# gersteinlab/LESSeq

Measured on AMD Instinct MI355X. Metric: MRF reads/sec through count+solve, higher is better.
Workload: dtype int32 coordinates / u64 counters (count), f64 (EM); 1 GPU; BASELINE configs[2]: 100M synthetic 100bp reads over 50k mixed events (SE/RI/A5SS/A3SS/MXE/AFE/ALE/T3), 24 chromosomes; events=50000

## Files before the change

### lesseq_amd/csrc/lsq_count.hip

```cpp
#include "lsq_device.hpp"
#include <hip/hip_ext.h>

namespace {

#ifndef LSQ_COUNT_BLOCK
#define LSQ_COUNT_BLOCK 256
#endif
constexpr int COUNT_BLOCK = LSQ_COUNT_BLOCK;
constexpr unsigned long long BASES_MASK = (1ull << 40) - 1;

#ifdef LSQ_DEV
#define ABL(args, bits) ((((args).ablate) & (bits)) != 0u)
#else
#define ABL(args, bits) false
#endif


struct CountArgs {
	const BucketDesc *buckets;
	const unsigned char *images;
	const TieRec *ties;
	const unsigned char *strand_rank;
	const char *read_names; const unsigned long long *read_name_off;
	const char *gene_names; const unsigned *gene_name_off;
// ... 1247 lines not shown
                     const unsigned *look1, const unsigned *look2, const size_t B, const unsigned long long grid, const SharePlanCosts &pc, unsigned long long *cut) {
	if (!(pc.weighted && pn1 && pn2 && look1 && look2)) { plan_share_cuts_seg(so, visited_kind, B, nullptr, nullptr, nullptr, nullptr, 0, grid, pc, cut); return; }
	std::vector<unsigned long long> x; std::vector<unsigned char> kind; std::vector<unsigned> looks, bseg(B + 1, 0);
	for (size_t b = 0; b < B; ++b) {
		bseg[b] = (unsigned)kind.size();
		const unsigned long long ns = so[b + 1] - so[b];
		if (!ns) continue;
		const bool visited = visited_kind[b] != 0;
		const unsigned long long n1 = visited ? std::min(pn1[b], ns) : 0, n2 = visited ? std::min(pn2[b], ns - n1) : 0;
		if (n1) { x.push_back(so[b]); kind.push_back(0); looks.push_back(look1[b]); }
		if (n2) { x.push_back(so[b] + n1); kind.push_back(1); looks.push_back(look2[b]); }
		if (ns - n1 - n2) { x.push_back(so[b] + n1 + n2); kind.push_back(2); looks.push_back(0); }
	}
	bseg[B] = (unsigned)kind.size();
	x.push_back(B ? so[B] : 0);
	plan_share_cuts_seg(so, visited_kind, B, x.data(), kind.data(), looks.data(), bseg.data(), kind.size(), grid, pc, cut);
}

int run_count(lsq_ctx *c) {
	const lsq_events &E = *c->E;
	const size_t n_cls = E.n_cls_total;
	const int M = E.n_methods;
	hipStream_t st_em = nullptr;
	const int set = c->flip ^ 1, other = c->flip;
	hipStream_t st = c->opt_two_count_streams ? c->stream_count2[set] : c->stream;
	if (c->mark_recorded2[set]) HIP_TRY(hipStreamWaitEvent(st, c->ev_mark2[set], 0));
	HIP_TRY(hipMemsetAsync(c->counters.p + (size_t)other * c->counters_per_set, 0, c->counters_per_set * sizeof(unsigned long long), c->stream_em2[other]));
	HIP_TRY(hipEventRecord(c->ev_mark2[other], c->stream_em2[other]));
	c->mark_recorded2[other] = true;
	select_counter_set(c, set);
	st_em = c->stream_em;
	c->fast_launched = 0;
	struct Cleanup { CountArgs A; unsigned long long n_pn; int m; };
	std::vector<Cleanup> cleanups;
	bool counted_signalled = false;
	if (c->time_events) HIP_TRY(hipEventRecord(c->ev0, st));
	const unsigned generic_tables_bytes = (std::max<unsigned>(E.max_lds_bytes, 16) + 15u) & ~15u;
	const unsigned tables_bytes = generic_tables_bytes;
	double max_skew = 0.0;
	for (int m = 0; m < M; ++m) max_skew = std::max(max_skew, c->reads[m].skew);
	const unsigned cap = c->opt_wg_per_cu >= 0 ? (unsigned)c->opt_wg_per_cu : (c->em.small_places >= c->em.opt_flat_min && max_skew < 4.0 ? 5u : 0u);
	const unsigned lds_bytes = std::max(tables_bytes + WAVES * WAVE_QUEUE_WORDS * 16, cap ? 160u * 1024u / (cap + 1u) + 16u : 0u);
	if (lds_bytes > 160 * 1024) return fail(LSQ_E_UNSUPPORTED, "bucket tables + read tile exceed the CU's LDS");
	bool all_compact = true;
	for (int m = 0; m < M; ++m) if (c->reads[m].total_slots && !c->reads[m].compact) all_compact = false;
	const int p1w = !all_compact ? 2 : (c->opt_reads_per_look ? (c->opt_reads_per_look == 8 ? 4 : 2) : (cap != 0 && cap <= 5 ? 4 : 2));
	const void *const fn_wide = (const void *)lsq_count_fast_kernel<false, 2>;
	const void *const fn_compact = p1w == 4 ? (const void *)lsq_count_fast_kernel<true, 4> : (const void *)lsq_count_fast_kernel<true, 2>;
	c->last_reads_per_look = 2u * (unsigned)p1w;
	if (lds_bytes > 64 * 1024) {
		HIP_TRY(hipFuncSetAttribute(fn_wide, hipFuncAttributeMaxDynamicSharedMemorySize, (int)lds_bytes));
		HIP_TRY(hipFuncSetAttribute(fn_compact, hipFuncAttributeMaxDynamicSharedMemorySize, (int)lds_bytes));
		HIP_TRY(hipFuncSetAttribute((const void *)lsq_count_generic_kernel, hipFuncAttributeMaxDynamicSharedMemorySize, (int)lds_bytes));
// ... 80 lines not shown
		A.exc = mr.exc.p + (size_t)set * mr.exc_cap; A.exc_count = c->exc_count.p + 2 * m; A.exc_cap = (unsigned)mr.exc_cap;
		A.dbg = c->dbg.p; A.bar = c->dbg.p + 16 + m;
		A.wg_trace = nullptr;
		const unsigned long long n_pn = mr.pn_strand.n;
		A.n_pn = n_pn;
		const unsigned workers_per_cu = 2;
		A.n_workers = (unsigned)std::min<unsigned long long>((n_pn + COUNT_BLOCK - 1) / COUNT_BLOCK, (unsigned long long)c->n_cu * workers_per_cu);
#ifdef LSQ_DEV
		if (c->dev_ablate & 32768u) A.n_workers = 0;
#endif
		if (c->has_fast) {
			if (c->time_events) HIP_TRY(hipEventRecord(c->evf0[m], st));
			const bool last_streaming = m == M - 1 && !c->has_generic && !c->time_events;
			const dim3 fgrid((unsigned)grid + A.n_workers);
#ifdef LSQ_DEV
			if (c->dev_ablate & 4194304u) {
				if (c->wg_trace.n < 4ull * fgrid.x) { int rc = c->wg_trace.alloc(4ull * fgrid.x); if (rc) return rc; }
				HIP_TRY(hipMemsetAsync(c->wg_trace.p, 0, 4ull * fgrid.x * sizeof(unsigned long long), st));
				c->wg_trace_n = fgrid.x; c->wg_trace_workers = A.n_workers;
				A.wg_trace = c->wg_trace.p;
			}
#endif
			void *kargs[] = {(void *)&A};
			HIP_TRY(hipExtLaunchKernel(mr.compact ? fn_compact : fn_wide, fgrid, dim3(COUNT_BLOCK), kargs, lds_bytes, st, nullptr, last_streaming ? c->ev_counted2[set] : nullptr, 0));
			if (last_streaming) counted_signalled = true;
			if (c->time_events) HIP_TRY(hipEventRecord(c->evf1[m], st));
			c->fast_launched |= 1 << m;
			cleanups.push_back({A, n_pn, m});
		}
		if (c->has_generic) {
			hipLaunchKernelGGL(lsq_count_generic_kernel, dim3((unsigned)grid), dim3(COUNT_BLOCK), generic_tables_bytes, st, A);
			HIP_TRY(hipGetLastError());
		}
	}
	if (c->time_events) HIP_TRY(hipEventRecord(c->ev1, st));
	c->count_timed = c->time_events;
	if (!counted_signalled) HIP_TRY(hipEventRecord(c->ev_counted2[set], st));
	HIP_TRY(hipStreamWaitEvent(st_em, c->ev_counted2[set], 0));
	const unsigned rgrid = std::max(16u, (unsigned)c->n_cu);
	if (c->recount_args.n < 2 * (size_t)LSQ_MAX_METHODS * sizeof(CountArgs)) {
		int rc = c->recount_args.alloc(2 * (size_t)LSQ_MAX_METHODS * sizeof(CountArgs));
		if (rc) return rc;
		c->recount_args_host.assign(2 * (size_t)LSQ_MAX_METHODS * sizeof(CountArgs), 0);
	}
	for (const Cleanup &u : cleanups) {
		const size_t slot = ((size_t)set * LSQ_MAX_METHODS + (size_t)u.m) * sizeof(CountArgs);
		if (memcmp(c->recount_args_host.data() + slot, &u.A, sizeof(CountArgs)) != 0) {
			memcpy(c->recount_args_host.data() + slot, &u.A, sizeof(CountArgs));
			HIP_TRY(hipMemcpyAsync(c->recount_args.p + slot, c->recount_args_host.data() + slot, sizeof(CountArgs), hipMemcpyHostToDevice, st_em));
		}
		const CountArgs *dA = reinterpret_cast<const CountArgs *>(c->recount_args.p + slot);
		hipLaunchKernelGGL(lsq_count_cleanup_kernel, dim3(c->opt_cleanup_grid ? c->opt_cleanup_grid : rgrid), dim3(256), 0, st_em, dA, c->opt_recount ? 1 : 0, u.n_pn,
		                   (const ExcEntry *)u.A.exc, (const unsigned *)u.A.exc_count, u.A.exc_cap);
		HIP_TRY(hipGetLastError());
	}
	return LSQ_OK;
}

}

extern "C" {

int lsq_count_status(lsq_ctx *c, uint32_t *exceptions, uint32_t *recounted) LSQ_API_TRY {
	if (!c) return fail(LSQ_E_ARG, "null context");
	if (!c->counted) return fail(LSQ_E_STATE, "lsq_count must come first");
	HIP_TRY(hipSetDevice(c->device));
// ... 78 lines not shown
```

### lesseq_amd/csrc/lsq_device.hip

```cpp
#include "lsq_device.hpp"
#include <chrono>
#include <thread>

namespace lsq {

int upload_strand_ranks(lsq_ctx *c) {
	const auto &names = c->E->strands.names;
	if (names.size() > 256) return fail(LSQ_E_RANGE, "more than 256 distinct strand strings");
	std::vector<int> order(names.size());
	std::iota(order.begin(), order.end(), 0);
	std::sort(order.begin(), order.end(), [&](int a, int b) { return names[a] < names[b]; });
	std::vector<uint8_t> rank(256, 0);
	for (size_t r = 0; r < order.size(); ++r) rank[order[r]] = (uint8_t)r;
	int rc = c->strand_rank.upload(rank.data(), 256, c->stream);
	if (rc) return rc;
	HIP_TRY(hipStreamSynchronize(c->stream));
	return LSQ_OK;
}

static hipError_t wait_for_stream(hipStream_t s) {
	const auto t0 = std::chrono::steady_clock::now();
	for (;;) {
		const hipError_t e = hipStreamQuery(s);
		if (e != hipErrorNotReady) return e;
		if (std::chrono::steady_clock::now() - t0 > std::chrono::milliseconds(2)) return hipStreamSynchronize(s);
	}
}

int ensure_lanes(lsq_ctx *c) {
	if (c->lanes_thread.joinable()) c->lanes_thread.join();
	if (c->lanes_status) return fail(c->lanes_status, "%s", c->lanes_error.c_str());
	return LSQ_OK;
}

int sync_all(lsq_ctx *c) {
	{ const int rc = ensure_lanes(c); if (rc) return rc; }
	HIP_TRY(wait_for_stream(c->stream_count2[0]));
	HIP_TRY(wait_for_stream(c->stream_count2[1]));
	HIP_TRY(wait_for_stream(c->stream_em2[0]));
	HIP_TRY(wait_for_stream(c->stream_em2[1]));
	HIP_TRY(wait_for_stream(c->stream));
	return LSQ_OK;
}

void select_counter_set(lsq_ctx *c, int set) {
	unsigned long long *base = c->counters.p + (size_t)set * c->counters_per_set;
	const size_t per = c->cnt.n;
	c->flip = set;
	c->stream_em = c->stream_em2[set];
	c->theta.p = c->theta2[set].p; c->theta.n = c->theta2[set].n;
	c->logll.p = c->logll2[set].p; c->logll.n = c->logll2[set].n;
	c->iters.p = c->iters2[set].p; c->iters.n = c->iters2[set].n;
	c->flags.p = c->flags2[set].p; c->flags.n = c->flags2[set].n;
	c->cnt.p = base;
	c->bases.p = base + per;
	c->exc_count.p = reinterpret_cast<unsigned *>(base + 2 * per);
	c->dbg.p = base + 2 * per + LSQ_MAX_METHODS;
}

void note_overflow(lsq_ctx *c, const std::vector<unsigned> &h) {
	for (int m = 0; m < c->E->n_methods; ++m) {
		if (!h[2 * (size_t)m + 1] || c->overflow_logged[m]) continue;
		c->overflow_logged[m] = true;
		if (c->opt_recount) continue;
		warn("read file %d: the exception list overflowed (%u pairs for %zu entries); every read of the file was counted again on the device. "
		     "Tables are complete; raise lsq_ctx_set_option \"exception_capacity\" to avoid the second pass", m, h[2 * (size_t)m], c->reads[m].exc_cap);
	}
}

}

extern "C" {

int lsq_ctx_create(int device_id, lsq_ctx **out) { return lsq_ctx_create_with(device_id, 0u, out); }

int lsq_ctx_create_with(int device_id, unsigned flags, lsq_ctx **out) LSQ_API_TRY {
	if (!out) return fail(LSQ_E_ARG, "null argument");
	const bool timing = getenv("LSQ_CLI_TIMING") != nullptr;
	auto t_last = std::chrono::steady_clock::now();
	auto mark = [&](const char *what) {
		if (!timing) return;
		const auto t = std::chrono::steady_clock::now();
		fprintf(stderr, "[timing]     %-32s %.3f s\n", what, std::chrono::duration<double>(t - t_last).count());
		t_last = t;
	};
	int n = 0;
	hipError_t e = hipGetDeviceCount(&n);
	mark("context: runtime start-up");
	if (e != hipSuccess || n <= 0) return fail(LSQ_E_DEVICE, "no HIP device available (%s)", e == hipSuccess ? "device count 0" : hipGetErrorString(e));
	if (device_id < 0 || device_id >= n) return fail(LSQ_E_ARG, "device %d out of range (%d devices)", device_id, n);
	HIP_TRY(hipSetDevice(device_id));
	hipDeviceProp_t prop;
	HIP_TRY(hipGetDeviceProperties(&prop, device_id));
	if (strncmp(prop.gcnArchName, "gfx950", 6) != 0)
		return fail(LSQ_E_DEVICE, "device %d is %s; this library carries gfx950 code only", device_id, prop.gcnArchName);
	mark("context: device selected");
	std::unique_ptr<lsq_ctx> c(new lsq_ctx);
	c->device = device_id;
	c->n_cu = prop.multiProcessorCount;
	HIP_TRY(hipStreamCreateWithFlags(&c->stream, hipStreamNonBlocking));
	HIP_TRY(hipEventCreate(&c->evt0)); HIP_TRY(hipEventCreate(&c->evt1));
	mark("context: upload stream");
	lsq_ctx *cp = c.get();
	auto make_lanes = [cp]() -> int {
		HIP_TRY(hipSetDevice(cp->device));
		for (int l = 0; l < 2; ++l) {
			HIP_TRY(hipStreamCreateWithFlags(&cp->stream_em2[l], hipStreamNonBlocking));
			HIP_TRY(hipStreamCreateWithFlags(&cp->stream_count2[l], hipStreamNonBlocking));
			HIP_TRY(hipEventCreateWithFlags(&cp->ev_counted2[l], hipEventDisableTiming));
			HIP_TRY(hipEventCreateWithFlags(&cp->ev_mark2[l], hipEventDisableTiming));
		}
		cp->stream_em = cp->stream_em2[0];
		HIP_TRY(hipEventCreate(&cp->ev0)); HIP_TRY(hipEventCreate(&cp->ev1));
		HIP_TRY(hipEventCreate(&cp->ev2)); HIP_TRY(hipEventCreate(&cp->ev3));
		for (int m = 0; m < LSQ_MAX_METHODS; ++m) { HIP_TRY(hipEventCreate(&cp->evf0[m])); HIP_TRY(hipEventCreate(&cp->evf1[m])); }
		return LSQ_OK;
	};
	if (flags & LSQ_CTX_LANES_IN_BACKGROUND) {
		c->lanes_thread = std::thread([cp, make_lanes]() noexcept {
			try { cp->lanes_status = make_lanes(); if (cp->lanes_status) cp->lanes_error = lsq_last_error(); }
			catch (...) { cp->lanes_status = LSQ_E_INTERNAL; try { cp->lanes_error = "the lanes' helper thread failed"; } catch (...) {} }
		});
	} else {
		const int rc = make_lanes();
		if (rc) return rc;
		mark("context: lanes");
	}
	*out = c.release();
	return LSQ_OK;
} LSQ_API_CATCH

void lsq_ctx_destroy(lsq_ctx *c) {
	if (!c) return;
	if (c->lanes_thread.joinable()) c->lanes_thread.join();
	(void)hipSetDevice(c->device);
	if (c->stream) (void)hipStreamSynchronize(c->stream);
	for (int l = 0; l < 2; ++l) {
		if (c->stream_em2[l]) (void)hipStreamSynchronize(c->stream_em2[l]);
		if (c->stream_count2[l]) (void)hipStreamSynchronize(c->stream_count2[l]);
		if (c->ev_counted2[l]) (void)hipEventDestroy(c->ev_counted2[l]);
		if (c->ev_mark2[l]) (void)hipEventDestroy(c->ev_mark2[l]);
	}
	if (c->ev0) (void)hipEventDestroy(c->ev0);
	if (c->ev1) (void)hipEventDestroy(c->ev1);
	if (c->ev2) (void)hipEventDestroy(c->ev2);
	if (c->ev3) (void)hipEventDestroy(c->ev3);
	if (c->evt0) (void)hipEventDestroy(c->evt0);
	if (c->evt1) (void)hipEventDestroy(c->evt1);
	for (int m = 0; m < LSQ_MAX_METHODS; ++m) { if (c->evf0[m]) (void)hipEventDestroy(c->evf0[m]); if (c->evf1[m]) (void)hipEventDestroy(c->evf1[m]); }
	for (IngestPass &p : c->ing_pass) for (hipEvent_t e : p.ev) if (e) (void)hipEventDestroy(e);
	for (int q = 0; q < 2; ++q) { if (c->pin_buf[q]) (void)hipHostFree(c->pin_buf[q]); if (c->pin_ev[q]) (void)hipEventDestroy(c->pin_ev[q]); }
	if (c->stream) (void)hipStreamDestroy(c->stream);
	for (int l = 0; l < 2; ++l) { if (c->stream_em2[l]) (void)hipStreamDestroy(c->stream_em2[l]); if (c->stream_count2[l]) (void)hipStreamDestroy(c->stream_count2[l]); }
	delete c;
}

void *lsq_ctx_stream(lsq_ctx *c) { return c ? (void *)c->stream : nullptr; }
int lsq_ctx_synchronize(lsq_ctx *c) LSQ_API_TRY {
	if (!c) return fail(LSQ_E_ARG, "null context");
	HIP_TRY(hipSetDevice(c->device));
	return sync_all(c);
} LSQ_API_CATCH

int lsq_ctx_synchronize_for(lsq_ctx *c, double seconds) LSQ_API_TRY {
	if (!c) return fail(LSQ_E_ARG, "null context");
// ... 85 lines not shown
			for (int j = 0; j < K; ++j) pi.push_back(E->dev_iso_base[dd] + (uint32_t)j);
			pe.push_back(dd);
		}
		if ((rc = c->pack_cls.upload(pc.data(), pc.size(), c->stream))) return rc;
		if ((rc = c->pack_iso.upload(pi.data(), pi.size(), c->stream))) return rc;
		if ((rc = c->pack_ev.upload(pe.data(), pe.size(), c->stream))) return rc;
	}
	mark("events: images, EM order, pack lists");
	const size_t n_iso = E->n_iso_total, M = (size_t)E->n_methods;
	std::vector<double> G(std::max<size_t>(M * n_iso, 1), 0.0);
	for (size_t d = 0; d < E->dev2out.size(); ++d) {
		const Event &ev = E->ev[E->dev2out[d]];
		for (size_t m = 0; m < M; ++m)
			for (int j = 0; j < ev.K; ++j) {
				double nd = (double)ev.ars[m][j];
				G[m * n_iso + E->dev_iso_base[d] + j] = nd <= 0 ? 0.0 : (double)1.0 / nd;
			}
	}
	if ((rc = c->G.upload(G.data(), M * n_iso, c->stream))) return rc;
	const size_t n_cls = E->n_cls_total, n_ev = E->dev2out.size();
	{
		const size_t per = std::max<size_t>(M, 1) * n_cls;
		c->counters_per_set = 2 * per + LSQ_MAX_METHODS + 16 + LSQ_MAX_METHODS;
		if ((rc = c->counters.alloc(2 * c->counters_per_set))) return rc;
		c->cnt.n = per; c->bases.n = per; c->exc_count.n = 2 * LSQ_MAX_METHODS; c->dbg.n = 16;
		c->mark_recorded2[0] = c->mark_recorded2[1] = false;
		c->fim_uploaded = false; c->fim_done = false;
		select_counter_set(c, 0);
		HIP_TRY(hipMemsetAsync(c->counters.p, 0, c->counters.n * sizeof(unsigned long long), c->stream));
	}
	for (int l = 0; l < 2; ++l) {
		if ((rc = c->theta2[l].alloc(n_iso)) || (rc = c->logll2[l].alloc(n_ev)) || (rc = c->iters2[l].alloc(n_ev)) || (rc = c->flags2[l].alloc(n_ev))) return rc;
		HIP_TRY(hipMemsetAsync(c->flags2[l].p, 0, std::max<size_t>(n_ev, 1), c->stream));
	}
	select_counter_set(c, 0);
	mark("events: G, counters, EM outputs");
	{
		const size_t nc = E->covered.size();
		std::vector<RouteChrom> chrom(std::max<size_t>(nc, 1));
		std::vector<int2> cov;
		std::vector<int4> clu;
		for (size_t ch = 0; ch < nc; ++ch) {
			RouteChrom &R = chrom[ch];
			memset(&R, 0, sizeof(R));
			R.cov0 = (unsigned)cov.size();
			for (size_t q = 0; q < E->covered[ch].s.size(); ++q) cov.push_back(make_int2((int)E->covered[ch].s[q], (int)E->covered[ch].e[q]));
			R.cov1 = (unsigned)cov.size();
			R.clu0 = (unsigned)clu.size();
			const int first = ch < E->chrom_first_bucket.size() ? E->chrom_first_bucket[ch] : -1;
			if (first >= 0 && ch < E->clu_s.size() && ch < E->cut_lo.size()) {
				const std::vector<int32_t> &cuts = E->cut_lo[ch];
				for (size_t q = 0; q < E->clu_s[ch].size(); ++q) {
					long long s = E->clu_s[ch][q];
					const long long e = E->clu_e[ch][q];
					while (s <= e) {
						const size_t ub = (size_t)(std::upper_bound(cuts.begin(), cuts.end(), (int32_t)s) - cuts.begin());
						const long long next_cut = ub < cuts.size() ? (long long)cuts[ub] : e + 1;
						const long long stop = std::min(e, next_cut - 1);
// ... 237 lines not shown
		for (size_t m = 0; m < M; ++m)
			for (size_t k = 0; k < nc; ++k) {
				hc[m * n_cls + E.dev_cls_base[d] + k] = class_count[m * n_out + E.class_off[o] + k];
				hb[m * n_cls + E.dev_cls_base[d] + k] = class_bases[m * n_out + E.class_off[o] + k];
			}
	}
	{ int rc = sync_all(c); if (rc) return rc; }
	if (M * n_cls) {
		HIP_TRY(hipMemcpyAsync(c->cnt.p, hc.data(), M * n_cls * sizeof(unsigned long long), hipMemcpyHostToDevice, c->stream));
		HIP_TRY(hipMemcpyAsync(c->bases.p, hb.data(), M * n_cls * sizeof(unsigned long long), hipMemcpyHostToDevice, c->stream));
		HIP_TRY(hipStreamSynchronize(c->stream));
	}
	c->counted = true; c->solved = false;
	c->counts_external = true;
	return LSQ_OK;
} LSQ_API_CATCH

uint64_t lsq_counts_device_words(const lsq_ctx *c) { return (c && c->E) ? 2ull * (uint64_t)c->E->n_methods * (uint64_t)c->E->n_cls_total : 0; }

int lsq_counts_export_device(lsq_ctx *c, void *d_words) LSQ_API_TRY {
	if (!c || !d_words) return fail(LSQ_E_ARG, "null argument");
	if (!c->counted) return fail(LSQ_E_STATE, "lsq_count must come first");
	HIP_TRY(hipSetDevice(c->device));
	const size_t per = (size_t)c->E->n_methods * c->E->n_cls_total;
	if (per) {
		HIP_TRY(hipMemcpyAsync(d_words, c->cnt.p, per * sizeof(unsigned long long), hipMemcpyDeviceToDevice, c->stream_em));
		HIP_TRY(hipMemcpyAsync((unsigned long long *)d_words + per, c->bases.p, per * sizeof(unsigned long long), hipMemcpyDeviceToDevice, c->stream_em));
	}
	return LSQ_OK;
} LSQ_API_CATCH

int lsq_counts_import_device(lsq_ctx *c, const void *d_words) LSQ_API_TRY {
	if (!c || !d_words) return fail(LSQ_E_ARG, "null argument");
	if (!c->E) return fail(LSQ_E_STATE, "lsq_events_upload must come first");
	HIP_TRY(hipSetDevice(c->device));
	const size_t per = (size_t)c->E->n_methods * c->E->n_cls_total;
	{ int rc = sync_all(c); if (rc) return rc; }
	if (per) {
		HIP_TRY(hipMemcpyAsync(c->cnt.p, d_words, per * sizeof(unsigned long long), hipMemcpyDeviceToDevice, c->stream_em));
		HIP_TRY(hipMemcpyAsync(c->bases.p, (const unsigned long long *)d_words + per, per * sizeof(unsigned long long), hipMemcpyDeviceToDevice, c->stream_em));
	}
	c->counted = true; c->solved = false;
	c->counts_external = true;
	return LSQ_OK;
} LSQ_API_CATCH

// ... 31 lines not shown
} LSQ_API_CATCH

}

namespace {
__global__ void __launch_bounds__(256) lsq_copy_results_kernel(unsigned long long *d0, const unsigned long long *s0, size_t n0, unsigned long long *d1,
                                                               const unsigned long long *s1, size_t n1, unsigned long long *d2, const unsigned long long *s2, size_t n2) {
	const size_t gsz = (size_t)gridDim.x * blockDim.x;
	for (size_t i = (size_t)blockIdx.x * blockDim.x + threadIdx.x; i < n0 + n1 + n2; i += gsz) {
		if (i < n0) d0[i] = s0[i];
		else if (i < n0 + n1) d1[i - n0] = s1[i - n0];
		else d2[i - n0 - n1] = s2[i - n0 - n1];
	}
}
}

extern "C" {

int lsq_results_copy_device(lsq_ctx *c, void *d_class_count, void *d_theta, void *d_logll) LSQ_API_TRY {
	if (!c) return fail(LSQ_E_ARG, "null context");
	if (!c->counted) return fail(LSQ_E_STATE, "lsq_count must come first");
	if ((d_theta || d_logll) && !c->solved) return fail(LSQ_E_STATE, "lsq_solve must come first");
	HIP_TRY(hipSetDevice(c->device));
	const lsq_events &E = *c->E;
	const size_t n_cls = E.n_cls_total, M = (size_t)E.n_methods;
	const size_t n0 = d_class_count ? M * n_cls : 0, n1 = d_theta ? (size_t)E.n_iso_total : 0, n2 = d_logll ? E.dev2out.size() : 0;
	if (n0 + n1 + n2) {
		const unsigned grid = (unsigned)std::min<size_t>((n0 + n1 + n2 + 255) / 256, (size_t)c->n_cu * 8);
		hipLaunchKernelGGL(lsq_copy_results_kernel, dim3(grid), dim3(256), 0, c->stream_em, (unsigned long long *)d_class_count, c->cnt.p, n0,
		                   (unsigned long long *)d_theta, (const unsigned long long *)c->theta.p, n1, (unsigned long long *)d_logll, (const unsigned long long *)c->logll.p, n2);
		HIP_TRY(hipGetLastError());
	}
	return LSQ_OK;
} LSQ_API_CATCH

extern "C++" {
namespace {
__global__ void __launch_bounds__(256) lsq_pack_results_kernel(unsigned long long *dst, const unsigned long long *cnt, const unsigned long long *bases,
                                                               const unsigned long long *theta, const unsigned long long *logll, const unsigned *pack_cls,
                                                               const unsigned *pack_iso, const unsigned *pack_ev, size_t M, size_t C, size_t I, size_t N,
                                                               size_t n_cls_dev) {
	const size_t total = 2 * M * C + I + N, gsz = (size_t)gridDim.x * blockDim.x;
	for (size_t i = (size_t)blockIdx.x * blockDim.x + threadIdx.x; i < total; i += gsz) {
		unsigned long long v;
		if (i < M * C) { const size_t m = i / C, k = i - m * C; v = cnt[m * n_cls_dev + pack_cls[k]]; }
		else if (i < 2 * M * C) { const size_t q = i - M * C, m = q / C, k = q - m * C; v = bases[m * n_cls_dev + pack_cls[k]]; }
		else if (i < 2 * M * C + I) v = theta[pack_iso[i - 2 * M * C]];
		else v = logll[pack_ev[i - 2 * M * C - I]];
		dst[i] = v;
	}
}
}
}

int lsq_results_pack_device(lsq_ctx *c, void *d_block) LSQ_API_TRY {
	if (!c || !d_block) return fail(LSQ_E_ARG, "null argument");
	if (!c->solved) return fail(LSQ_E_STATE, "lsq_solve must come first");
	HIP_TRY(hipSetDevice(c->device));
	const lsq_events &E = *c->E;
	const size_t M = (size_t)E.n_methods, C = c->pack_cls.n, I = c->pack_iso.n, N = c->pack_ev.n;
	const size_t total = 2 * M * C + I + N;
	if (total) {
		const unsigned grid = (unsigned)std::min<size_t>((total + 255) / 256, (size_t)c->n_cu * 8);
		hipLaunchKernelGGL(lsq_pack_results_kernel, dim3(grid), dim3(256), 0, c->stream_em, (unsigned long long *)d_block, c->cnt.p, c->bases.p,
		                   (const unsigned long long *)c->theta.p, (const unsigned long long *)c->logll.p, c->pack_cls.p, c->pack_iso.p, c->pack_ev.p, M, C, I, N,
		                   (size_t)E.n_cls_total);
		HIP_TRY(hipGetLastError());
	}
	return LSQ_OK;
} LSQ_API_CATCH

void *lsq_ctx_result_stream(lsq_ctx *c) { return c ? (void *)c->stream_em : nullptr; }

int lsq_device_alloc(lsq_ctx *c, uint64_t bytes, void **out) LSQ_API_TRY {
	if (!c || !out) return fail(LSQ_E_ARG, "null argument");
	HIP_TRY(hipSetDevice(c->device));
	HIP_TRY(hipMalloc(out, (size_t)std::max<uint64_t>(bytes, 8)));
	HIP_TRY(hipMemsetAsync(*out, 0, (size_t)std::max<uint64_t>(bytes, 8), c->stream_em));
	HIP_TRY(hipStreamSynchronize(c->stream_em));
	return LSQ_OK;
} LSQ_API_CATCH
void lsq_device_free(lsq_ctx *c, void *p) {
	if (!c || !p) return;
	(void)hipSetDevice(c->device);
	(void)hipFree(p);
}
int lsq_device_write(lsq_ctx *c, void *device_dst, const void *host_src, uint64_t bytes) LSQ_API_TRY {
	if (!c || !device_dst || !host_src) return fail(LSQ_E_ARG, "null argument");
	HIP_TRY(hipSetDevice(c->device));
	{ int rc = sync_all(c); if (rc) return rc; }
	HIP_TRY(hipMemcpy(device_dst, host_src, (size_t)bytes, hipMemcpyHostToDevice));
	return LSQ_OK;
} LSQ_API_CATCH
int lsq_device_read(lsq_ctx *c, void *host_dst, const void *device_src, uint64_t bytes) LSQ_API_TRY {
	if (!c || !host_dst || !device_src) return fail(LSQ_E_ARG, "null argument");
	HIP_TRY(hipSetDevice(c->device));
	{ int rc = sync_all(c); if (rc) return rc; }
	HIP_TRY(hipMemcpy(host_dst, device_src, (size_t)bytes, hipMemcpyDeviceToHost));
	return LSQ_OK;
// ... 116 lines not shown
		else c->opt_share_taper = value;
		for (auto &r : c->reads) r.wg_grid = 0;
	} else if (n == "sam_skip_flags") {
		if (!(value >= 0 && value <= 65535)) return fail(LSQ_E_ARG, "sam_skip_flags must lie in 0..65535");
		c->opt_sam_skip_flags = (unsigned)value;
	} else if (n == "sam_min_mapq") {
		if (!(value >= 0 && value <= 256)) return fail(LSQ_E_ARG, "sam_min_mapq must lie in 0..256");
		c->opt_sam_min_mapq = (unsigned)value;
	} else if (n == "bam_verify") {
		if (!(value == 0 || value == 1)) return fail(LSQ_E_ARG, "bam_verify must be 0 or 1");
		c->opt_bam_verify = value == 1;
	} else if (n == "compact_pools") {
		c->opt_compact_pools = value != 0;
	} else if (n == "workgroups_per_cu") {
		if (!(value >= -1 && value <= 32)) return fail(LSQ_E_ARG, "workgroups_per_cu must lie in -1..32 (-1 = automatic, 0 = as many as fit)");
		c->opt_wg_per_cu = (int)value;
		c->occ_lds_bytes = 0;
	} else if (n == "reads_per_look") {
		if (!(value == 0 || value == 4 || value == 8)) return fail(LSQ_E_ARG, "reads_per_look must be 0 (automatic), 4 or 8");
		c->opt_reads_per_look = (int)value;
	} else if (n == "count_streams") {
		{ int rc = sync_all(c); if (rc) return rc; }
		c->opt_two_count_streams = value >= 2;
	} else if (n == "em_flat_min_events") {
		if (!(value >= 0 && value <= 4e9)) return fail(LSQ_E_ARG, "em_flat_min_events must lie in 0..4e9");
		c->em.opt_flat_min = (unsigned)value;
	} else if (n == "em_closed_form") {
		{ int rc = sync_all(c); if (rc) return rc; }
		c->em.opt_closed = value != 0;
	} else if (n == "em_quad_cap") {
		if (value < 0 || value > 1e6) return fail(LSQ_E_ARG, "em_quad_cap out of range");
		c->em.opt_quad_cap = (unsigned)value;
	} else if (n == "bootstrap_chunk") {
		if (!(value >= 0 && value <= 4096)) return fail(LSQ_E_ARG, "bootstrap_chunk must lie in 0..4096 (0 = automatic)");
		c->boot.opt_chunk = (unsigned)value;
	} else if (n == "em_regroup") {
		c->em.opt_regroup = value != 0;
		for (EmLane &l : c->em.lane) l.order_valid = false;
	} else if (n == "recount_every_read") {
		c->opt_recount = value != 0;
	} else if (n == "cleanup_workgroups") {
		if (value < 0 || value > 4096) return fail(LSQ_E_ARG, "cleanup_workgroups out of range");
		c->opt_cleanup_grid = (unsigned)value;
	} else if (n == "em_guard_band") {
		return lsq_set_em_guard_band(c, value);
	} else
// ... 33 lines not shown
```

### lesseq_amd/csrc/lsq_device.hpp

```cpp
#pragma once
#include <hip/hip_runtime.h>

#include <algorithm>
#include <cmath>
#include <cstring>
#include <memory>
#include <numeric>
#include <string>
#include <thread>
#include <type_traits>
#include <vector>

#include "lsq_internal.hpp"

using namespace lsq;

#define HIP_TRY(expr)                                                                          \
	do {                                                                                       \
		hipError_t _e = (expr);                                                                \
		if (_e != hipSuccess) return fail(LSQ_E_DEVICE, "%s: %s", #expr, hipGetErrorString(_e)); \
	} while (0)


#ifndef LSQ_P1_PAD
#define LSQ_P1_PAD 8
#endif
#ifndef LSQ_P2_PAD
#define LSQ_P2_PAD 4
#endif
constexpr unsigned P2_GROUP_PAD = LSQ_P2_PAD;
constexpr unsigned P1_GROUP_PAD = LSQ_P1_PAD;
constexpr int LSQ_INGEST_STAGES = 7;
constexpr int LSQ_INGEST_PASS_MAX = 16;
constexpr int EM_LANES = 4;

namespace lsq {

constexpr unsigned COMPACT_OFF_BITS = 22, COMPACT_OFF_MASK = (1u << COMPACT_OFF_BITS) - 1u, COMPACT_MAX_LEN = 1u << 10;
constexpr int COMPACT_BIAS = 1 << 21;
__host__ __device__ inline bool compact_block_fits(long long off, long long len) { return off >= 0 && off <= (long long)COMPACT_OFF_MASK && len > 0 && len < (long long)COMPACT_MAX_LEN; }

struct ExcEntry {
	unsigned long long slot;
	unsigned bucket;
	unsigned ev_pool_scan;
};

template <class T>
struct DevBuf {
	T *p = nullptr;
	size_t n = 0;
	~DevBuf() { if (p) (void)hipFree(p); }
	int alloc(size_t count) {
		if (p) { (void)hipFree(p); p = nullptr; }
		n = count;
		HIP_TRY(hipMalloc((void **)&p, std::max<size_t>(count, 1) * sizeof(T)));
// ... 128 lines not shown
	lsq::DevBuf<double> theta;
	lsq::DevBuf<double> stats;
	lsq::DevBuf<uint32_t> n_ok;
	unsigned B = 0;
	bool done = false;
	unsigned opt_chunk = 0;
	unsigned last_chunk = 0;
	float ms[3] = {0, 0, 0};
	bool timed = false;
};

struct lsq_ctx {
	std::thread lanes_thread;
	int lanes_status = 0;
	std::string lanes_error;
	int device = 0;
	int n_cu = 256;
	hipStream_t stream = nullptr;
	hipStream_t stream_em = nullptr;
	hipStream_t stream_em2[2] = {nullptr, nullptr};
	hipStream_t stream_count2[2] = {nullptr, nullptr};
	bool opt_two_count_streams = true;
	int opt_wg_per_cu = -1;
	hipEvent_t ev_counted2[2] = {nullptr, nullptr}, ev_mark2[2] = {nullptr, nullptr};
	bool mark_recorded2[2] = {false, false};
	int flip = 0;
	size_t counters_per_set = 0;
	hipEvent_t ev0 = nullptr, ev1 = nullptr, ev2 = nullptr, ev3 = nullptr;
	hipEvent_t evt0 = nullptr, evt1 = nullptr;
	hipEvent_t evf0[LSQ_MAX_METHODS] = {}, evf1[LSQ_MAX_METHODS] = {};
	int fast_launched = 0;
	int occ_p1w = 0;
	int opt_reads_per_look = 0;
	unsigned last_reads_per_look = 4, last_wg_per_cu = 0;
	unsigned occ_lds_bytes = 0; int occ_blocks = 0;
	bool time_events = false;
	bool count_timed = false, solve_timed = false;
	lsq_events *E = nullptr;
	DevBuf<BucketDesc> buckets;
	DevBuf<uint8_t> images, strand_rank, dK;
	DevBuf<TieRec> ties;
	DevBuf<uint32_t> cls_base, iso_base, gene_name_off;
	DevBuf<char> gene_names;
	DevBuf<uint32_t> pack_cls, pack_iso, pack_ev;
	EmState em;
	BootState boot;
	DevBuf<double> G, theta2[2], logll2[2];
	DevBuf<uint32_t> iters2[2];
	DevBuf<uint8_t> flags2[2];
// ... 60 lines not shown

struct lsq_text {
	std::string path;
	unsigned long long offset = 0, len = 0;
	lsq::DevBuf<unsigned char> d_text;
	float h2d_ms = 0;
	bool scanned = false;
	unsigned long long n_nl = 0;
	lsq::DevBuf<unsigned long long> d_tile_base;
};

namespace lsq {
int upload_strand_ranks(lsq_ctx *c);
int run_count(lsq_ctx *c);
int run_solve(lsq_ctx *c);
int run_fim(lsq_ctx *c);
int run_boot_em(lsq_ctx *c, unsigned n_rep, const unsigned long long *cnt, double *theta, double *logll, unsigned *iters, unsigned char *flags);
int sync_all(lsq_ctx *c);
int ensure_lanes(lsq_ctx *c);
void note_overflow(lsq_ctx *c, const std::vector<unsigned> &exc_count);
int host_count(lsq_ctx *c);
int host_solve(lsq_ctx *c);
int replay_flagged(lsq_ctx *c, unsigned *n_done);
void select_counter_set(lsq_ctx *c, int set);
}
```

### lesseq_amd/csrc/lsq_em.hip

```cpp
#include "lsq_device.hpp"

namespace {

struct EmArgs {
	unsigned n_events, n_methods, n_cls, n_iso;
	unsigned n_places;
	unsigned place0;
	double band;
	unsigned max_iters;
	const unsigned *order;
	const unsigned *split;
	const unsigned char *K;
	const unsigned *cls_base, *iso_base;
	const unsigned long long *cnt;
	const double *G;
	double *theta, *logll;
	unsigned *iters;
	unsigned char *flags;
};


template <int CTRL>
__device__ inline double quad_perm_f64(double x) {
	int lo = __double2loint(x), hi = __double2hiint(x);
// ... 719 lines not shown
}

static int schedule_regroup(lsq_ctx *c, const int lane, const bool flat) {
	EmState &S = c->em;
	EmLane &L = S.lane[lane];
	if (!S.opt_regroup || (L.order_valid && ++L.age < 16)) return LSQ_OK;
	L.age = 0;
	S.last.regrouped = true;
	if (flat) {
		HIP_TRY(hipMemcpyAsync(S.split.p + EM_SPLIT_KEPT, S.split.p + lane, sizeof(uint32_t), hipMemcpyDeviceToDevice, c->stream_em));
		S.last.split_word = EM_SPLIT_KEPT;
	}
	if (L.order.n != S.small_places) { int rc = L.order.alloc(S.small_places); if (rc) return rc; }
	hipLaunchKernelGGL(lsq_em_regroup_kernel, dim3(1), dim3(1024), 0, c->stream_em, S.order.p, c->iters.p, S.small_places, L.order.p, S.split.p + lane);
	HIP_TRY(hipGetLastError());
	L.order_valid = true;
	return LSQ_OK;
}

static int launch_lean(lsq_ctx *c, EmArgs A) {
	const lsq_events &E = *c->E;
	EmState &S = c->em;
	hipStream_t st = c->stream_em;
	const int lane = c->flip;
	const unsigned blk = 64, np = S.small_places, n_lane_wg = (np + blk - 1) / blk;
	A.place0 = 0; A.n_places = np;
	if (S.opt_closed && E.n_methods == 1) {
		const EmTail T = em_tail_of(c, lane);
		hipLaunchKernelGGL(lsq_em_head_kernel<3>, dim3(n_lane_wg), dim3(blk), 0, st, A, T);
		hipLaunchKernelGGL(lsq_em_tail_kernel<3>, dim3(n_lane_wg), dim3(blk), 0, st, A, T);
		HIP_TRY(hipGetLastError());
		S.last.form = EM_FORM_HEAD_TAIL; S.last.lean = np;
		return LSQ_OK;
	}
	const bool regrouped = S.opt_regroup && S.lane[lane].order_valid;
	if (regrouped) A.order = S.lane[lane].order.p;
	const bool flat = regrouped && np >= S.opt_flat_min;
	const unsigned split_word = flat ? (unsigned)lane : EM_SPLIT_NONE;
	A.split = S.split.p + split_word;
	const unsigned n_quad = (np * EM_LANES + blk - 1) / blk, n_flat = flat ? n_lane_wg : 0u;
	const bool capped = !flat && S.opt_quad_cap && E.n_methods == 1;
	if (capped) {
		const EmTail T = em_tail_of(c, lane);
		hipLaunchKernelGGL(lsq_em_lean_quad_capped_kernel, dim3(n_quad), dim3(blk), 0, st, A, T, S.opt_quad_cap);
		hipLaunchKernelGGL(lsq_em_tail_kernel<3>, dim3(n_lane_wg), dim3(blk), 0, st, A, T);
	} else if (!flat) hipLaunchKernelGGL(lsq_em_lean_quad_kernel, dim3(n_quad), dim3(blk), 0, st, A);
	else if (E.n_methods == 1) hipLaunchKernelGGL(lsq_em_lean_kernel<3>, dim3(n_quad + n_flat), dim3(blk), 0, st, A, n_quad);
	else hipLaunchKernelGGL(lsq_em_lean_kernel<4>, dim3(n_quad + n_flat), dim3(blk), 0, st, A, n_quad);
	HIP_TRY(hipGetLastError());
	S.last.form = capped ? EM_FORM_QUAD_CAPPED : !flat ? EM_FORM_QUAD : E.n_methods == 1 ? EM_FORM_QUAD_FLAT3 : EM_FORM_QUAD_FLAT4;
	S.last.cap = capped ? S.opt_quad_cap : 0u;
	S.last.lean = np; S.last.learnt = regrouped; S.last.split_word = split_word;
	return schedule_regroup(c, lane, flat);
}

static int launch_general(lsq_ctx *c, EmArgs A) {
	A.place0 = c->em.small_places; A.n_places = c->em.places;
	const unsigned n = A.n_places - A.place0;
	hipLaunchKernelGGL(lsq_em_kernel, dim3((n * EM_LANES + 255) / 256), dim3(256), 0, c->stream_em, A);
	HIP_TRY(hipGetLastError());
	c->em.last.general = n;
	return LSQ_OK;
}

int run_solve(lsq_ctx *c) {
	const lsq_events &E = *c->E;
	hipStream_t st = c->stream_em;
	if (c->time_events) HIP_TRY(hipEventRecord(c->ev2, st));
	const unsigned n_ev = (unsigned)E.dev2out.size();
	c->em.last = {};
	c->em.last.lane = (unsigned)c->flip;
	if (n_ev) {
		EmArgs A{};
		A.n_events = n_ev; A.n_methods = (unsigned)E.n_methods; A.n_cls = E.n_cls_total; A.n_iso = E.n_iso_total;
		A.K = c->dK.p; A.cls_base = c->cls_base.p; A.iso_base = c->iso_base.p;
		A.order = c->em.order.p;
		A.max_iters = 1000000u;
		A.band = c->em_band;
#ifdef LSQ_DEV
		if (const char *e = getenv("LSQ_EM_CAP")) { const int v = atoi(e); if (v > 0) A.max_iters = (unsigned)v; }
#endif
		A.cnt = c->cnt.p; A.G = c->G.p; A.theta = c->theta.p; A.logll = c->logll.p; A.iters = c->iters.p; A.flags = c->flags.p;
		int rc = LSQ_OK;
		if (c->em.small_places && (rc = launch_lean(c, A))) return rc;
		if (c->em.places > c->em.small_places && (rc = launch_general(c, A))) return rc;
	}
	if (c->time_events) HIP_TRY(hipEventRecord(c->ev3, st));
	c->solve_timed = c->time_events;
	return LSQ_OK;
}

int run_boot_em(lsq_ctx *c, unsigned n_rep, const unsigned long long *cnt, double *theta, double *logll, unsigned *iters, unsigned char *flags) {
	const lsq_events &E = *c->E;
	const unsigned n_ev = (unsigned)E.dev2out.size();
// ... 28 lines not shown
```

### lesseq_amd/csrc/lsq_ingest.hip

```cpp
#include "lsq_ingest.hpp"
#include "lsq_text.hpp"

namespace {

struct IngestRaw {
	unsigned long long n_reads;
	const unsigned long long *blk_off;
	const unsigned *line_no;
	const int *blk_start, *blk_end;
	const unsigned short *blk_chrom;
	const unsigned char *blk_strand;
};

#ifndef LSQ_RAW_WAVES
#define LSQ_RAW_WAVES 8
#endif
template <bool STRANDED, class... Lib>
__global__ void __launch_bounds__(256) __attribute__((amdgpu_waves_per_eu(LSQ_RAW_WAVES))) lsq_route_raw_kernel(RouteTables T, IngestRaw R, RouteOut O, Lib... lib_arg) {
	__shared__ RouteChrom chrom_lds[ROUTE_CHROM_LDS];
	const RouteChrom *chroms = route_stage_chroms(T, chrom_lds);
	const unsigned long long gsz = (unsigned long long)gridDim.x * blockDim.x;
	LocProbe P;
	P.chrom = -1; P.bin = 0;
	if constexpr (!STRANDED) {
// ... 583 lines not shown
			hipLaunchKernelGGL(lsq_group_place_kernel, dim3((unsigned)n_pieces), dim3(256), place_lds, st, P);
		}
		if (FC + FJ) {
			const unsigned pgrid = (unsigned)std::min<size_t>((FC + FJ) / 256 + 1, (size_t)c->n_cu * 8);
			hipLaunchKernelGGL(lsq_ingest_pad_kernel, dim3(pgrid), dim3(256), 0, st, c->buckets.p, c->cell_base.p, c->jgroup_base.p, B, (unsigned)FC, (unsigned)FJ,
			                   (const unsigned *)cnt1, (const unsigned long long *)d_off1.p, (const unsigned *)cnt2, (const unsigned long long *)d_off2.p, c->images.p,
			                   (void *)mr.p1.p, (void *)mr.p2.p, compact, mr.p1_strand.p, mr.p1_line.p, mr.p2_strand.p, mr.p2_line.p);
		}
		if (nn) {
			NbOut N{};
			N.ent = d_nb_ent.p; N.blk = d_nb_blk.p; N.n_ent = nb_tot[0]; N.pn_off = mr.pn_off.p; N.pnb_off = mr.pnb_off.p; N.curn = curn; N.curnb = curnb;
			N.pn_blk_off = mr.pn_blk_off.p; N.pn_nblk = mr.pn_nblk.p; N.pn_line = mr.pn_line.p; N.pn_bucket = mr.pn_bucket.p; N.pn_strand = mr.pn_strand.p;
			N.pn_se = reinterpret_cast<int2 *>(mr.pn_se.p); N.line_no = F.line_no; N.first_line = F.first_line;
			const unsigned ngrid = (unsigned)std::min<unsigned long long>((nb_tot[0] + 255) / 256, (unsigned long long)c->n_cu * 16);
			hipLaunchKernelGGL(lsq_ingest_nblock_kernel, dim3(ngrid), dim3(256), 0, st, N);
		}
		HIP_TRY(hipGetLastError());
		k.end(16ull * n1p + 32ull * n2p + 4ull * (n1p + n2p) + (mr.compact ? 4ull : 8ull) * (n1 + 2 * n2) + 5ull * (n1 + n2));
	}
	{
		size_t want = std::max<size_t>(65536, (n1 + n2) / 4);
		if (c->opt_exc_cap) want = c->opt_exc_cap;
		if (mr.exc_cap != want) {
			if ((rc = mr.exc.alloc(2 * want))) return rc;
			mr.exc_cap = want;
		}
	}
	if ((rc = upload_strand_ranks(c))) return rc;
	mr.n_retained = tot[0];
	for (int q = 0; q < 5; ++q) {
		mr.lib_report[q] = 0;
		for (size_t k = 0; k < lib_places.size(); k += 8) mr.lib_report[q] += lib_places[k + q];
	}
	mr.n_retained_blocks = tot[1] + nb_tot[1];
	mr.total_slots = n1 + n2 + nn;
	mr.wg_grid = 0;
	{
		std::vector<unsigned long long> so(B + 1, 0), o1(B + 1, 0), o2(B + 1, 0), f1(FC + 1, 0), f2(FJ + 1, 0);
		std::vector<unsigned> park(FC + FJ + 1, 0);
		HIP_TRY(hipMemcpyAsync(so.data(), mr.slot_off.p, (B + 1) * sizeof(unsigned long long), hipMemcpyDeviceToHost, st));
		HIP_TRY(hipMemcpyAsync(o1.data(), mr.p1_off.p, (B + 1) * sizeof(unsigned long long), hipMemcpyDeviceToHost, st));
		HIP_TRY(hipMemcpyAsync(o2.data(), mr.p2_off.p, (B + 1) * sizeof(unsigned long long), hipMemcpyDeviceToHost, st));
		HIP_TRY(hipMemcpyAsync(f1.data(), d_off1.p, (FC + 1) * sizeof(unsigned long long), hipMemcpyDeviceToHost, st));
		HIP_TRY(hipMemcpyAsync(f2.data(), d_off2.p, (FJ + 1) * sizeof(unsigned long long), hipMemcpyDeviceToHost, st));
		if (FC + FJ) HIP_TRY(hipMemcpyAsync(park.data(), park1, (FC + FJ) * sizeof(unsigned), hipMemcpyDeviceToHost, st));
		HIP_TRY(hipStreamSynchronize(st));
		SW.mark("ingest: place + read-back");
// ... 172 lines not shown
```

Before: 741.2 billion reads/s.

## Triple-buffer counter sets so zeroing and EM overlap more count passes

Decouples the counter-set index from the stream lane and rotates through three counter sets instead of two. The memset of the previously used set then has a full extra iteration to finish before that set is reused, which removes a wait where a count pass blocks on zeroing. Lane streams are now created before the upload stream unless background creation is requested, in which case only two sets are used. The cost is more device memory for counters and exception buffers, plus more complex event bookkeeping.

```diff
diff --git a/lesseq_amd/csrc/lsq_count.hip b/lesseq_amd/csrc/lsq_count.hip
--- a/lesseq_amd/csrc/lsq_count.hip
+++ b/lesseq_amd/csrc/lsq_count.hip
@@ -1293,13 +1293,14 @@
 	const size_t n_cls = E.n_cls_total;
 	const int M = E.n_methods;
 	hipStream_t st_em = nullptr;
-	const int set = c->flip ^ 1, other = c->flip;
-	hipStream_t st = c->opt_two_count_streams ? c->stream_count2[set] : c->stream;
+	const int prev_lane = c->lane, prev_set = c->set;
+	const int lane = prev_lane ^ 1, set = (prev_set + 1) % c->opt_counter_sets;
+	hipStream_t st = c->opt_two_count_streams ? c->stream_count2[lane] : c->stream;
 	if (c->mark_recorded2[set]) HIP_TRY(hipStreamWaitEvent(st, c->ev_mark2[set], 0));
-	HIP_TRY(hipMemsetAsync(c->counters.p + (size_t)other * c->counters_per_set, 0, c->counters_per_set * sizeof(unsigned long long), c->stream_em2[other]));
-	HIP_TRY(hipEventRecord(c->ev_mark2[other], c->stream_em2[other]));
-	c->mark_recorded2[other] = true;
-	select_counter_set(c, set);
+	HIP_TRY(hipMemsetAsync(c->counters.p + (size_t)prev_set * c->counters_per_set, 0, c->counters_per_set * sizeof(unsigned long long), c->stream_em2[prev_lane]));
+	HIP_TRY(hipEventRecord(c->ev_mark2[prev_set], c->stream_em2[prev_lane]));
+	c->mark_recorded2[prev_set] = true;
+	select_counter_set(c, lane, set);
 	st_em = c->stream_em;
 	c->fast_launched = 0;
 	struct Cleanup { CountArgs A; unsigned long long n_pn; int m; };
@@ -1426,7 +1427,7 @@
 			}
 #endif
 			void *kargs[] = {(void *)&A};
-			HIP_TRY(hipExtLaunchKernel(mr.compact ? fn_compact : fn_wide, fgrid, dim3(COUNT_BLOCK), kargs, lds_bytes, st, nullptr, last_streaming ? c->ev_counted2[set] : nullptr, 0));
+			HIP_TRY(hipExtLaunchKernel(mr.compact ? fn_compact : fn_wide, fgrid, dim3(COUNT_BLOCK), kargs, lds_bytes, st, nullptr, last_streaming ? c->ev_counted2[lane] : nullptr, 0));
 			if (last_streaming) counted_signalled = true;
 			if (c->time_events) HIP_TRY(hipEventRecord(c->evf1[m], st));
 			c->fast_launched |= 1 << m;
@@ -1439,13 +1440,13 @@
 	}
 	if (c->time_events) HIP_TRY(hipEventRecord(c->ev1, st));
 	c->count_timed = c->time_events;
-	if (!counted_signalled) HIP_TRY(hipEventRecord(c->ev_counted2[set], st));
-	HIP_TRY(hipStreamWaitEvent(st_em, c->ev_counted2[set], 0));
+	if (!counted_signalled) HIP_TRY(hipEventRecord(c->ev_counted2[lane], st));
+	HIP_TRY(hipStreamWaitEvent(st_em, c->ev_counted2[lane], 0));
 	const unsigned rgrid = std::max(16u, (unsigned)c->n_cu);
-	if (c->recount_args.n < 2 * (size_t)LSQ_MAX_METHODS * sizeof(CountArgs)) {
-		int rc = c->recount_args.alloc(2 * (size_t)LSQ_MAX_METHODS * sizeof(CountArgs));
+	if (c->recount_args.n < (size_t)LSQ_COUNTER_SETS * LSQ_MAX_METHODS * sizeof(CountArgs)) {
+		int rc = c->recount_args.alloc((size_t)LSQ_COUNTER_SETS * LSQ_MAX_METHODS * sizeof(CountArgs));
 		if (rc) return rc;
-		c->recount_args_host.assign(2 * (size_t)LSQ_MAX_METHODS * sizeof(CountArgs), 0);
+		c->recount_args_host.assign((size_t)LSQ_COUNTER_SETS * LSQ_MAX_METHODS * sizeof(CountArgs), 0);
 	}
 	for (const Cleanup &u : cleanups) {
 		const size_t slot = ((size_t)set * LSQ_MAX_METHODS + (size_t)u.m) * sizeof(CountArgs);
diff --git a/lesseq_amd/csrc/lsq_device.hip b/lesseq_amd/csrc/lsq_device.hip
--- a/lesseq_amd/csrc/lsq_device.hip
+++ b/lesseq_amd/csrc/lsq_device.hip
@@ -43,15 +43,16 @@
 	return LSQ_OK;
 }
 
-void select_counter_set(lsq_ctx *c, int set) {
+void select_counter_set(lsq_ctx *c, int lane, int set) {
 	unsigned long long *base = c->counters.p + (size_t)set * c->counters_per_set;
 	const size_t per = c->cnt.n;
-	c->flip = set;
-	c->stream_em = c->stream_em2[set];
-	c->theta.p = c->theta2[set].p; c->theta.n = c->theta2[set].n;
-	c->logll.p = c->logll2[set].p; c->logll.n = c->logll2[set].n;
-	c->iters.p = c->iters2[set].p; c->iters.n = c->iters2[set].n;
-	c->flags.p = c->flags2[set].p; c->flags.n = c->flags2[set].n;
+	c->lane = lane;
+	c->set = set;
+	c->stream_em = c->stream_em2[lane];
+	c->theta.p = c->theta2[lane].p; c->theta.n = c->theta2[lane].n;
+	c->logll.p = c->logll2[lane].p; c->logll.n = c->logll2[lane].n;
+	c->iters.p = c->iters2[lane].p; c->iters.n = c->iters2[lane].n;
+	c->flags.p = c->flags2[lane].p; c->flags.n = c->flags2[lane].n;
 	c->cnt.p = base;
 	c->bases.p = base + per;
 	c->exc_count.p = reinterpret_cast<unsigned *>(base + 2 * per);
@@ -98,9 +99,6 @@
 	std::unique_ptr<lsq_ctx> c(new lsq_ctx);
 	c->device = device_id;
 	c->n_cu = prop.multiProcessorCount;
-	HIP_TRY(hipStreamCreateWithFlags(&c->stream, hipStreamNonBlocking));
-	HIP_TRY(hipEventCreate(&c->evt0)); HIP_TRY(hipEventCreate(&c->evt1));
-	mark("context: upload stream");
 	lsq_ctx *cp = c.get();
 	auto make_lanes = [cp]() -> int {
 		HIP_TRY(hipSetDevice(cp->device));
@@ -108,20 +106,33 @@
 			HIP_TRY(hipStreamCreateWithFlags(&cp->stream_em2[l], hipStreamNonBlocking));
 			HIP_TRY(hipStreamCreateWithFlags(&cp->stream_count2[l], hipStreamNonBlocking));
 			HIP_TRY(hipEventCreateWithFlags(&cp->ev_counted2[l], hipEventDisableTiming));
-			HIP_TRY(hipEventCreateWithFlags(&cp->ev_mark2[l], hipEventDisableTiming));
 		}
+		for (hipEvent_t &e : cp->ev_mark2) HIP_TRY(hipEventCreateWithFlags(&e, hipEventDisableTiming));
 		cp->stream_em = cp->stream_em2[0];
 		HIP_TRY(hipEventCreate(&cp->ev0)); HIP_TRY(hipEventCreate(&cp->ev1));
 		HIP_TRY(hipEventCreate(&cp->ev2)); HIP_TRY(hipEventCreate(&cp->ev3));
 		for (int m = 0; m < LSQ_MAX_METHODS; ++m) { HIP_TRY(hipEventCreate(&cp->evf0[m])); HIP_TRY(hipEventCreate(&cp->evf1[m])); }
 		return LSQ_OK;
 	};
+	bool lanes_first = !(flags & LSQ_CTX_LANES_IN_BACKGROUND);
+#ifdef LSQ_DEV
+	if (getenv("LSQ_UPLOAD_STREAM_FIRST")) lanes_first = false;
+#endif
+	if (lanes_first) {
+		const int rc = make_lanes();
+		if (rc) return rc;
+		mark("context: lanes");
+	} else
+		c->opt_counter_sets = 2;
+	HIP_TRY(hipStreamCreateWithFlags(&c->stream, hipStreamNonBlocking));
+	HIP_TRY(hipEventCreate(&c->evt0)); HIP_TRY(hipEventCreate(&c->evt1));
+	mark("context: upload stream");
 	if (flags & LSQ_CTX_LANES_IN_BACKGROUND) {
 		c->lanes_thread = std::thread([cp, make_lanes]() noexcept {
 			try { cp->lanes_status = make_lanes(); if (cp->lanes_status) cp->lanes_error = lsq_last_error(); }
 			catch (...) { cp->lanes_status = LSQ_E_INTERNAL; try { cp->lanes_error = "the lanes' helper thread failed"; } catch (...) {} }
 		});
-	} else {
+	} else if (!lanes_first) {
 		const int rc = make_lanes();
 		if (rc) return rc;
 		mark("context: lanes");
@@ -139,8 +150,8 @@
 		if (c->stream_em2[l]) (void)hipStreamSynchronize(c->stream_em2[l]);
 		if (c->stream_count2[l]) (void)hipStreamSynchronize(c->stream_count2[l]);
 		if (c->ev_counted2[l]) (void)hipEventDestroy(c->ev_counted2[l]);
-		if (c->ev_mark2[l]) (void)hipEventDestroy(c->ev_mark2[l]);
-	}
+	}
+	for (hipEvent_t e : c->ev_mark2) if (e) (void)hipEventDestroy(e);
 	if (c->ev0) (void)hipEventDestroy(c->ev0);
 	if (c->ev1) (void)hipEventDestroy(c->ev1);
 	if (c->ev2) (void)hipEventDestroy(c->ev2);
@@ -272,18 +283,18 @@
 	{
 		const size_t per = std::max<size_t>(M, 1) * n_cls;
 		c->counters_per_set = 2 * per + LSQ_MAX_METHODS + 16 + LSQ_MAX_METHODS;
-		if ((rc = c->counters.alloc(2 * c->counters_per_set))) return rc;
+		if ((rc = c->counters.alloc(LSQ_COUNTER_SETS * c->counters_per_set))) return rc;
 		c->cnt.n = per; c->bases.n = per; c->exc_count.n = 2 * LSQ_MAX_METHODS; c->dbg.n = 16;
-		c->mark_recorded2[0] = c->mark_recorded2[1] = false;
+		for (bool &r : c->mark_recorded2) r = false;
 		c->fim_uploaded = false; c->fim_done = false;
-		select_counter_set(c, 0);
+		select_counter_set(c, 0, 0);
 		HIP_TRY(hipMemsetAsync(c->counters.p, 0, c->counters.n * sizeof(unsigned long long), c->stream));
 	}
 	for (int l = 0; l < 2; ++l) {
 		if ((rc = c->theta2[l].alloc(n_iso)) || (rc = c->logll2[l].alloc(n_ev)) || (rc = c->iters2[l].alloc(n_ev)) || (rc = c->flags2[l].alloc(n_ev))) return rc;
 		HIP_TRY(hipMemsetAsync(c->flags2[l].p, 0, std::max<size_t>(n_ev, 1), c->stream));
 	}
-	select_counter_set(c, 0);
+	select_counter_set(c, 0, 0);
 	mark("events: G, counters, EM outputs");
 	{
 		const size_t nc = E->covered.size();
@@ -567,6 +578,7 @@
 	if (!c || !d_words) return fail(LSQ_E_ARG, "null argument");
 	if (!c->counted) return fail(LSQ_E_STATE, "lsq_count must come first");
 	HIP_TRY(hipSetDevice(c->device));
+	{ int rc = ensure_lanes(c); if (rc) return rc; }
 	const size_t per = (size_t)c->E->n_methods * c->E->n_cls_total;
 	if (per) {
 		HIP_TRY(hipMemcpyAsync(d_words, c->cnt.p, per * sizeof(unsigned long long), hipMemcpyDeviceToDevice, c->stream_em));
@@ -644,6 +656,7 @@
 	if (!c->counted) return fail(LSQ_E_STATE, "lsq_count must come first");
 	if ((d_theta || d_logll) && !c->solved) return fail(LSQ_E_STATE, "lsq_solve must come first");
 	HIP_TRY(hipSetDevice(c->device));
+	{ int rc = ensure_lanes(c); if (rc) return rc; }
 	const lsq_events &E = *c->E;
 	const size_t n_cls = E.n_cls_total, M = (size_t)E.n_methods;
 	const size_t n0 = d_class_count ? M * n_cls : 0, n1 = d_theta ? (size_t)E.n_iso_total : 0, n2 = d_logll ? E.dev2out.size() : 0;
@@ -679,6 +692,7 @@
 	if (!c || !d_block) return fail(LSQ_E_ARG, "null argument");
 	if (!c->solved) return fail(LSQ_E_STATE, "lsq_solve must come first");
 	HIP_TRY(hipSetDevice(c->device));
+	{ int rc = ensure_lanes(c); if (rc) return rc; }
 	const lsq_events &E = *c->E;
 	const size_t M = (size_t)E.n_methods, C = c->pack_cls.n, I = c->pack_iso.n, N = c->pack_ev.n;
 	const size_t total = 2 * M * C + I + N;
@@ -692,11 +706,12 @@
 	return LSQ_OK;
 } LSQ_API_CATCH
 
-void *lsq_ctx_result_stream(lsq_ctx *c) { return c ? (void *)c->stream_em : nullptr; }
+void *lsq_ctx_result_stream(lsq_ctx *c) { return (c && ensure_lanes(c) == LSQ_OK) ? (void *)c->stream_em : nullptr; }
 
 int lsq_device_alloc(lsq_ctx *c, uint64_t bytes, void **out) LSQ_API_TRY {
 	if (!c || !out) return fail(LSQ_E_ARG, "null argument");
 	HIP_TRY(hipSetDevice(c->device));
+	{ int rc = ensure_lanes(c); if (rc) return rc; }
 	HIP_TRY(hipMalloc(out, (size_t)std::max<uint64_t>(bytes, 8)));
 	HIP_TRY(hipMemsetAsync(*out, 0, (size_t)std::max<uint64_t>(bytes, 8), c->stream_em));
 	HIP_TRY(hipStreamSynchronize(c->stream_em));
@@ -859,6 +874,16 @@
 	} else if (n == "count_streams") {
 		{ int rc = sync_all(c); if (rc) return rc; }
 		c->opt_two_count_streams = value >= 2;
+	} else if (n == "counter_sets") {
+		if (!(value == 2 || value == LSQ_COUNTER_SETS)) return fail(LSQ_E_ARG, "counter_sets must be 2 or %d", LSQ_COUNTER_SETS);
+		{ int rc = ensure_lanes(c); if (rc) return rc; }
+		HIP_TRY(hipSetDevice(c->device));
+		for (const hipStream_t q : {c->stream_count2[0], c->stream_count2[1], c->stream_em2[0], c->stream_em2[1], c->stream}) {
+			const hipError_t e = hipStreamQuery(q);
+			if (e == hipErrorNotReady) return fail(LSQ_E_STATE, "counter_sets may only be set while nothing is in flight (lsq_ctx_synchronize first)");
+			if (e != hipSuccess) return fail(LSQ_E_DEVICE, "hipStreamQuery: %s", hipGetErrorString(e));
+		}
+		c->opt_counter_sets = (int)value;
 	} else if (n == "em_flat_min_events") {
 		if (!(value >= 0 && value <= 4e9)) return fail(LSQ_E_ARG, "em_flat_min_events must lie in 0..4e9");
 		c->em.opt_flat_min = (unsigned)value;
diff --git a/lesseq_amd/csrc/lsq_device.hpp b/lesseq_amd/csrc/lsq_device.hpp
--- a/lesseq_amd/csrc/lsq_device.hpp
+++ b/lesseq_amd/csrc/lsq_device.hpp
@@ -32,6 +32,7 @@
 constexpr unsigned P1_GROUP_PAD = LSQ_P1_PAD;
 constexpr int LSQ_INGEST_STAGES = 7;
 constexpr int LSQ_INGEST_PASS_MAX = 16;
+constexpr int LSQ_COUNTER_SETS = 3;
 constexpr int EM_LANES = 4;
 
 namespace lsq {
@@ -206,9 +207,11 @@
 	hipStream_t stream_count2[2] = {nullptr, nullptr};
 	bool opt_two_count_streams = true;
 	int opt_wg_per_cu = -1;
-	hipEvent_t ev_counted2[2] = {nullptr, nullptr}, ev_mark2[2] = {nullptr, nullptr};
-	bool mark_recorded2[2] = {false, false};
-	int flip = 0;
+	hipEvent_t ev_counted2[2] = {nullptr, nullptr}, ev_mark2[LSQ_COUNTER_SETS] = {};
+	bool mark_recorded2[LSQ_COUNTER_SETS] = {};
+	int lane = 0;
+	int set = 0;
+	int opt_counter_sets = LSQ_COUNTER_SETS;
 	size_t counters_per_set = 0;
 	hipEvent_t ev0 = nullptr, ev1 = nullptr, ev2 = nullptr, ev3 = nullptr;
 	hipEvent_t evt0 = nullptr, evt1 = nullptr;
@@ -315,5 +318,5 @@
 int host_count(lsq_ctx *c);
 int host_solve(lsq_ctx *c);
 int replay_flagged(lsq_ctx *c, unsigned *n_done);
-void select_counter_set(lsq_ctx *c, int set);
+void select_counter_set(lsq_ctx *c, int lane, int set);
 }
diff --git a/lesseq_amd/csrc/lsq_em.hip b/lesseq_amd/csrc/lsq_em.hip
--- a/lesseq_amd/csrc/lsq_em.hip
+++ b/lesseq_amd/csrc/lsq_em.hip
@@ -765,7 +765,7 @@
 	const lsq_events &E = *c->E;
 	EmState &S = c->em;
 	hipStream_t st = c->stream_em;
-	const int lane = c->flip;
+	const int lane = c->lane;
 	const unsigned blk = 64, np = S.small_places, n_lane_wg = (np + blk - 1) / blk;
 	A.place0 = 0; A.n_places = np;
 	if (S.opt_closed && E.n_methods == 1) {
@@ -812,7 +812,7 @@
 	if (c->time_events) HIP_TRY(hipEventRecord(c->ev2, st));
 	const unsigned n_ev = (unsigned)E.dev2out.size();
 	c->em.last = {};
-	c->em.last.lane = (unsigned)c->flip;
+	c->em.last.lane = (unsigned)c->lane;
 	if (n_ev) {
 		EmArgs A{};
 		A.n_events = n_ev; A.n_methods = (unsigned)E.n_methods; A.n_cls = E.n_cls_total; A.n_iso = E.n_iso_total;
diff --git a/lesseq_amd/csrc/lsq_ingest.hip b/lesseq_amd/csrc/lsq_ingest.hip
--- a/lesseq_amd/csrc/lsq_ingest.hip
+++ b/lesseq_amd/csrc/lsq_ingest.hip
@@ -629,7 +629,7 @@
 		size_t want = std::max<size_t>(65536, (n1 + n2) / 4);
 		if (c->opt_exc_cap) want = c->opt_exc_cap;
 		if (mr.exc_cap != want) {
-			if ((rc = mr.exc.alloc(2 * want))) return rc;
+			if ((rc = mr.exc.alloc(LSQ_COUNTER_SETS * want))) return rc;
 			mr.exc_cap = want;
 		}
 	}
```

Result: faster. 836.6 billion reads/s (median of 6 runs) (+12.9%).
